# simon-donike/NIR-GAN

Hardware: AMD Instinct MI355X
Metric: 256x256 RGB tiles/sec (G+D fwd+bwd+step) (higher is better)
Workload: dtype f32 (3xbf16 split, 6 products, f32 accumulate) for the contractions with 32-channel runs incl. the Winograd plane GEMMs; exact f32 MFMA for the first / last layers; f32 everywhere else; 1 GPU; configs[1]: 6-block ResnetGenerator + 3-layer PatchGAN, bs=16/GPU, 256x256, GAN+L1, padding=0, fp32-equivalent MFMA (three bf16 terms, six products); global_batch=16, parallelism=dp1

## Files before the change

### nir-gan_amd/csrc/igemm_conv.hip

```cpp
#include "igemm_tiles.h"
#include "igemm_tile256.h"
#include "igemm_x3.h"
#include <cstdlib>
#include "igemm_x3r.h"

namespace {

template <int BN, int PREC = 0, bool WB16 = false, bool AB16 = false>
__global__ __launch_bounds__(256, 2) void conv_igemm_kernel(const ng::ConvParams p) {
    __shared__ __attribute__((aligned(16))) char st0[(128 + BN) * 128];
    __shared__ __attribute__((aligned(16))) char st1[(128 + BN) * 128];
    ng::conv_tile<BN, PREC, WB16, AB16>(p, blockIdx.x, st0, st1);
}

__global__ __launch_bounds__(512, 2) void conv_igemm256_kernel(const ng::ConvParams p) {
    __shared__ __attribute__((aligned(16))) char lds[ng::T256_LDS];
    ng::conv_tile256(p, ng_xcd_remap(blockIdx.x, gridDim.x), lds);
}

template <int BN>
__global__ __launch_bounds__(512, 2) void conv_x3_kernel(const ng::X3Work w) {
    __shared__ __attribute__((aligned(16))) char sA0[ng::X3_A_BYTES];
    __shared__ __attribute__((aligned(16))) char sA1[ng::X3_A_BYTES];
    __shared__ __attribute__((aligned(16))) char sB0[3 * BN * 64];
// ... 51 lines not shown
    int k = 0;
    if (bid >= g.first[1]) k = 1;
    if (bid >= g.first[2]) k = 2;
    if (bid >= g.first[3]) k = 3;
    if (k == 0) ng::conv_tile<BN, PREC, WB16, AB16>(g.p[0], bid, st0, st1);
    else if (k == 1) ng::conv_tile<BN, PREC, WB16, AB16>(g.p[1], bid - g.first[1], st0, st1);
    else if (k == 2) ng::conv_tile<BN, PREC, WB16, AB16>(g.p[2], bid - g.first[2], st0, st1);
    else ng::conv_tile<BN, PREC, WB16, AB16>(g.p[3], bid - g.first[3], st0, st1);
}

}

int ng::ng_cu_count_conv() {
    static int cus = 0;
    if (cus == 0) {
        int dev = 0, n = 0;
        if (hipGetDevice(&dev) != hipSuccess || hipDeviceGetAttribute(&n, hipDeviceAttributeMultiprocessorCount, dev) != hipSuccess || n <= 0) n = 256;
        cus = n;
#ifdef NG_X3R_STAMP
        if (const char* e = getenv("NG_X3R_CUS")) cus = atoi(e);
#endif
    }
    return cus;
}
using ng::ng_cu_count_conv;

int ng::ng_launch_conv_x3(const ng::ConvParams* ps, const int n, const int bn, const int nplanes, const long long in_plane, const long long w3_pstride,
                          const long long out_plane, hipStream_t st, const char* what) {
    ng::X3Work w;
    int total = 0;
    for (int i = 0; i < n; ++i) { w.p[i] = ps[i]; w.first[i] = total; total += ng::conv_x3_tiles(ps[i], bn) * (nplanes > 1 ? nplanes : 1); }
    for (int i = n; i < 4; ++i) { w.p[i] = ps[0]; w.first[i] = 0x7fffffff; }
    w.first[n] = total;
    for (int i = n + 1; i < 5; ++i) w.first[i] = 0x7fffffff;
    w.n = n;
    w.nplanes = nplanes > 1 ? nplanes : 1;
    w.in_plane = in_plane; w.w3_pstride = w3_pstride; w.out_plane = out_plane;
    w.spread = 0;
    for (int i = 0; i < 4; ++i) w.start[i] = 0;
    const int G = ng_cu_count_conv();
    bool unequal = false;
    for (int i = 1; i < n; ++i) unequal = unequal || ps[i].K != ps[0].K;
    if (n >= 2 && w.nplanes == 1 && unequal && total >= G && G <= 1024) {
        long long load[2 * 1024 + 1];
        for (int i = 0; i < G; ++i) load[i] = 0;
        int order[4] = {0, 1, 2, 3};
        for (int i = 0; i < n; ++i)
            for (int j = i + 1; j < n; ++j)
                if (ps[order[j]].K > ps[order[i]].K) { const int t = order[i]; order[i] = order[j]; order[j] = t; }
        for (int oi = 0; oi < n; ++oi) {
            const int k = order[oi];
            const int rem = (w.first[k + 1] - w.first[k]) % G;
            if (rem == 0) continue;
            const long long cost = ps[k].K / 32 + 3;
            long long prefix[2 * 1024 + 1];
            prefix[0] = 0;
            for (int i = 0; i < 2 * G; ++i) prefix[i + 1] = prefix[i] + load[i % G];
            int best = 0;
            for (int s0 = 1; s0 < G; ++s0)
                if (prefix[s0 + rem] - prefix[s0] < prefix[best + rem] - prefix[best]) best = s0;
            for (int t = 0; t < rem; ++t) load[(best + t) % G] += cost;
            w.start[k] = best;
        }
        w.spread = 1;
    }
    const dim3 grid(total < G ? total : G);
    switch (ng::conv_x3_route(ps, n, bn)) {
        case ng::X3R_GENERIC: hipLaunchKernelGGL((conv_x3r_kernel<128, 2>), grid, dim3(256), 0, st, w); break;
        case ng::X3R_STATS: hipLaunchKernelGGL((conv_x3r_kernel<128, 1>), grid, dim3(256), 0, st, w); break;
        case ng::X3R_PLAIN: hipLaunchKernelGGL((conv_x3r_kernel<128, 0>), grid, dim3(256), 0, st, w); break;
        case ng::X3_N128: hipLaunchKernelGGL(conv_x3_kernel<128>, grid, dim3(512), 0, st, w); break;
        case ng::X3_N64: hipLaunchKernelGGL(conv_x3_kernel<64>, grid, dim3(512), 0, st, w); break;
    }
    return nirgan_check_launch(what);
}

ng::X3Kernel ng::conv_x3_route(const ng::ConvParams* ps, const int n, const int bn) {
    bool reg_fed = true, gen = false, stats = false;
    for (int i = 0; i < n; ++i) {
        reg_fed = reg_fed && ng::conv_x3r_ok(ps[i], bn);
        gen = gen || ng::conv_x3r_generic(ps[i]);
        stats = stats || ng::conv_x3r_stats(ps[i]);
    }
    if (reg_fed) return gen ? ng::X3R_GENERIC : (stats ? ng::X3R_STATS : ng::X3R_PLAIN);
    return bn == 128 ? ng::X3_N128 : ng::X3_N64;
}

enum ConvKernel { CONV_K_X3R, CONV_K_X3_N128, CONV_K_X3_N64, CONV_K_TILE256, CONV_K_TILE128, CONV_K_TILE64 };
static const char* const CONV_KERNEL_NAMES[] = {"conv_x3r_kernel<128>", "conv_x3_kernel<128>", "conv_x3_kernel<64>", "conv_igemm256_kernel",
                                                "conv_igemm_kernel<128>", "conv_igemm_kernel<64>"};
struct ConvRoute { ConvKernel k; int bn; };
static ConvRoute conv_route(const ng::ConvParams* ps, const int n, const bool group) {
    bool x3 = ps[0].prec == 3;
    for (int i = 0; i < n; ++i) x3 = x3 && ng::conv_x3_ok(ps[i]) && (ps[i].N % 128 == 0) == (ps[0].N % 128 == 0);
    if (x3) {
        const int bn = ng::conv_x3_bn(ps, n, ng_cu_count_conv());
        const ng::X3Kernel k = ng::conv_x3_route(ps, n, bn);
        return {k == ng::X3_N128 ? CONV_K_X3_N128 : (k == ng::X3_N64 ? CONV_K_X3_N64 : CONV_K_X3R), bn};
    }
    if (!group && ps[0].algo != NIRGAN_CONV_TILE128 && ng::conv_tile256_ok(ps[0])) return {CONV_K_TILE256, 0};
    return {ps[0].N > 64 ? CONV_K_TILE128 : CONV_K_TILE64, 0};
}
static bool conv_route_x3(const ConvRoute& r) { return r.k == CONV_K_X3R || r.k == CONV_K_X3_N128 || r.k == CONV_K_X3_N64; }

#ifdef NG_X3R_STAMP
extern "C" int nirgan_x3r_stamps(unsigned long long* host, int n) {
    return hipMemcpyFromSymbol(host, HIP_SYMBOL(ng::ng_x3r_stamps), size_t(n) * 8) == hipSuccess ? 0 : -1;
}
#endif

extern "C" int nirgan_split3(const float* src, void* dst_bf16, int64_t n, int64_t plane, void* stream) {
    NG_REQUIRE(src && dst_bf16 && n > 0 && n % 8 == 0 && plane >= n && plane % 8 == 0, "split3: n and plane must be positive multiples of 8, plane >= n");
    NG_REQUIRE(ng_aligned16(src) && ng_aligned16(dst_bf16), "split3: pointers must be 16-byte aligned");
    hipLaunchKernelGGL(split3_kernel, dim3((unsigned)((n / 8 + 255) / 256)), dim3(256), 0, static_cast<hipStream_t>(stream),
                       src, static_cast<unsigned short*>(dst_bf16), (long long)n, (long long)plane);
    return nirgan_check_launch("split3");
}

extern "C" int nirgan_conv_igemm(const nirgan_conv_desc* d, void* stream) {
    ng::ConvParams p;
    const int rc = ng::build_conv_params(d, p);
    if (rc != NIRGAN_OK) return rc;
    hipStream_t st = static_cast<hipStream_t>(stream);
    const ConvRoute r = conv_route(&p, 1, false);
    if (conv_route_x3(r)) return ng::ng_launch_conv_x3(&p, 1, r.bn, 1, 0, 0, 0, st, "conv_igemm (three-term split tile)");
    if (p.prec == 3) {
        NG_REQUIRE(p.ch == p.N, "conv: out_span = 2 needs a problem the three-term split tile covers (run %% 32 == 0, N %% 64 == 0)");
        p.prec = 0;
    }
    if (r.k == CONV_K_TILE256) {
        hipLaunchKernelGGL(conv_igemm256_kernel, dim3(((p.M + 255) >> 8) * (p.N >> 8)), dim3(512), 0, st, p);
        return nirgan_check_launch("conv_igemm (256 x 256 tile)");
    }
    const dim3 grid(p.mtiles * p.ntiles * p.ksplit);
    ng::conv_tile_form(p, [&](auto form) {
        using F = decltype(form);
        if (r.k == CONV_K_TILE128) hipLaunchKernelGGL((conv_igemm_kernel<128, F::prec, F::wb16, F::ab16>), grid, dim3(256), 0, st, p);
        else hipLaunchKernelGGL((conv_igemm_kernel<64, F::prec, F::wb16, F::ab16>), grid, dim3(256), 0, st, p);
    });
    if (p.ksplit > 1) {
        const long long total = (long long)p.M * (p.N / 4);
        const int grid = int((total + 255) / 256 < 4096 ? (total + 255) / 256 : 4096);
        hipLaunchKernelGGL(conv_splitk_reduce_kernel, dim3(grid), dim3(256), 0, st, p);
    }
    return nirgan_check_launch("conv_igemm");
}

extern "C" const char* nirgan_conv_kernel_name(const nirgan_conv_desc* d) {
    ng::ConvParams p;
    if (ng::build_conv_params(d, p) != NIRGAN_OK) return nullptr;
    return CONV_KERNEL_NAMES[conv_route(&p, 1, false).k];
}

extern "C" int nirgan_conv_igemm_group(const nirgan_conv_desc* const* descs, int n, void* stream) {
    NG_REQUIRE(descs != nullptr && n >= 1 && n <= 4, "conv_igemm_group: 1..4 descriptors");
    ConvGroup g;
    int total = 0;
    bool wide = false;
    for (int i = 0; i < n; ++i) {
        NG_REQUIRE(descs[i] != nullptr, "conv_igemm_group: null descriptor %d", i);
        const int rc = ng::build_conv_params(descs[i], g.p[i]);
        if (rc != NIRGAN_OK) return rc;
        NG_REQUIRE(descs[i]->ksplit <= 1, "conv_igemm_group: split-K descriptors are not groupable");
        const bool w = descs[i]->N > 64;
        NG_REQUIRE(i == 0 || w == wide, "conv_igemm_group: all problems must use the same tile width (N <= 64 or N > 64)");
        NG_REQUIRE(g.p[i].prec == g.p[0].prec && g.p[i].w_bf16 == g.p[0].w_bf16 && g.p[i].in_bf16 == g.p[0].in_bf16, "conv_igemm_group: all problems must use the same precision and weight storage");
        wide = w;
// ... 23 lines not shown
```

### nir-gan_amd/csrc/igemm_x3r.h

```cpp
#pragma once
#include "igemm_x3.h"

namespace ng {

#ifdef NG_X3R_STAMP
__device__ unsigned long long ng_x3r_stamps[1024 * 4 * 16];
#define X3R_STAMP(k) { unsigned long long t_; __builtin_amdgcn_sched_barrier(0); asm volatile("s_memtime %0\n\ts_waitcnt lgkmcnt(0)" : "=s"(t_) :: "memory"); \
                       __builtin_amdgcn_sched_barrier(0); st_sum[k] += unsigned(t_) - st_last; st_last = unsigned(t_); }
#else
#define X3R_STAMP(k)
#endif

template <int BN>
struct X3R {
    static constexpr int NT = BN / 16;
    static constexpr int B_TERM = BN * 64;
    static constexpr int STAGE = 3 * B_TERM;
    static constexpr int NSTAGE = 2;
    static constexpr int RING = NSTAGE * STAGE;
    static constexpr int STG = 2 * 16 * BN * 4;
    static constexpr int BPT = BN / 16;
    static constexpr int PIECES = 3 * BPT / 4;
    static constexpr int LPR = BN / 4;
    static constexpr int RPP = 64 / LPR;
// ... 360 lines not shown
            asm volatile(X3R_WAITL X3R_PAIR(MA, MA, T, "", "", X3R_ST0, X3R_ST1, "") : X3R_ACC, X3R_B_INOUT, X3R_TERMS : X3R_A_IN, [w] "n"(WAIT), X3R_ST_IN : CLOB); \
        } else if constexpr (WAIT >= 0) { \
            asm volatile(X3R_WAITL X3R_PAIR(MA, MA, T, "", "", "", "", "") : X3R_ACC, X3R_B_INOUT, X3R_TERMS : X3R_A_IN, [w] "n"(WAIT) : CLOB); \
        } else if constexpr (LB) { \
            const char* const lb = P == 0 ? baseW[0] : (P == 1 ? baseW[1] : baseW[2]); \
            const unsigned lo0 = L.b0, lo1 = L.b1; \
            asm volatile(X3R_PAIR(MA, MA, T, "", "", X3R_LB0, X3R_LB1, "") : X3R_ACC, X3R_TERMS, X3R_LB_OUT : X3R_A_IN, X3R_B_IN, [lo0] "v"(lo0), [lo1] "v"(lo1), [lb] "s"(lb) : CLOB); \
        } else if constexpr (LA) { \
            const char* const lb = base; \
            asm volatile(X3R_PAIR(MA, MA, T, "", "", X3R_LA0, X3R_LA1, "") : X3R_ACC, X3R_TERMS, X3R_LA_OUT : X3R_A_IN, X3R_B_IN, [lo0] "v"(goff), [lb] "s"(lb) : CLOB); \
        } else if constexpr (PR) { \
            asm volatile(X3R_PAIR(MA, MA, T, X3R_PR0, X3R_PR1, X3R_PR2, "", "") : X3R_ACC, X3R_TERMS, X3R_PR_OUT : X3R_A_IN, X3R_B_IN, X3R_PR_IN : CLOB); \
        } else { \
            asm volatile(X3R_PAIR(MA, MA, T, "", "", "", "", "") : X3R_ACC, X3R_TERMS : X3R_A_IN, X3R_B_IN : CLOB); \
        }
        if constexpr (P & 1) {
            if constexpr (FIRST) { X3R_EMIT(X3R_MZ, X3R_TB, X3R_CLOB_B) } else { X3R_EMIT(X3R_MC, X3R_TB, X3R_CLOB_B) }
        } else {
            if constexpr (FIRST) { X3R_EMIT(X3R_MZ, X3R_TA, X3R_CLOB_A) } else { X3R_EMIT(X3R_MC, X3R_TA, X3R_CLOB_A) }
        }
#undef X3R_EMIT
#undef X3R_ACC
#undef X3R_B_INOUT
#undef X3R_B_IN
#undef X3R_TERMS
#undef X3R_A_IN
#undef X3R_PR_OUT
#undef X3R_PR_IN
#undef X3R_ST_IN
#undef X3R_LB_OUT
#undef X3R_LA_OUT
        A[SRC][0][P] = h;
        A[SRC][1][P] = m;
        A[SRC][2][P] = l;
    };
#define X3R_RB(NTI, ad) { X3R_DSR(Bf[NTI][0], ad, (NTI) * 1024); X3R_DSR(Bf[NTI][1], ad, B_TERM + (NTI) * 1024); X3R_DSR(Bf[NTI][2], ad, 2 * B_TERM + (NTI) * 1024); }

    struct Slot {
        const NG_CONST ConvParams* p;
        float* out;
        int m0, n0, nk;
    };
    Slot E;
    char* const stg8 = stg_all + wave * T::STG;
    float* const stg = reinterpret_cast<float*>(stg8);
    const unsigned stg_lds = unsigned(size_t((NG_LDS char*)stg8));
    const int chunk = lane % LPR, lrow = lane / LPR;
    struct Epi {
        int pM, OHW, OW, OH, out_img, out_row, out_px, out_org, f_img, f_row, f_px, f_org, pC, span;
        const float* f_y;
        bool fused, stats;
        float fneg;
        int n, nq, nc, m, b, oh, ow, fb, mbase;
        f32x4 bv, fm, fr, s1, s2;
        float k0[NT], t1[NT], t2[NT];
    };
    auto epi_begin = [&](Epi& e) {
#pragma unroll
        for (int nt = 0; nt < NT; ++nt) e.k0[nt] = e.t1[nt] = e.t2[nt] = 0.f;
        const NG_CONST ConvParams& p = *E.p;
        e.pM = p.M; e.OHW = p.OHW; e.OW = p.OW; e.OH = p.OHW / p.OW; e.out_img = p.out_img; e.out_row = p.out_row * p.out_stride;
        e.out_px = p.out_cs * p.out_stride; e.out_org = p.out_org; e.f_img = p.f_img; e.f_row = p.f_row * p.out_stride; e.f_px = p.ch * p.out_stride;
        e.f_org = p.f_org; e.pC = p.ch; e.span = p.N / p.ch;
        e.f_y = p.f_y;
        e.mbase = E.m0 + wave * 64;
        e.fused = e.f_y != nullptr;
        e.stats = p.stats != nullptr && e.mbase < e.pM;
        e.fneg = p.f_act == NIRGAN_ACT_RELU ? 0.f : (p.f_act == NIRGAN_ACT_LRELU ? p.f_slope : 1.f);
        e.n = E.n0 + chunk * 4;
        e.bv = f32x4{0.f, 0.f, 0.f, 0.f};
        if (p.bias != nullptr) {
            const char* bb = ng_uniform_ptr(reinterpret_cast<const char*>(p.bias));
            const unsigned bo = unsigned(e.n) * 4u;
            asm volatile("global_load_dwordx4 %0, %1, %2\n\ts_waitcnt vmcnt(0)" : "=&v"(e.bv) : "v"(bo), "s"(bb) : "memory");
        }
        e.m = e.mbase + lrow;
        const int mc = e.m < e.pM ? e.m : e.pM - 1;
        split_row(mc, e.OHW, e.OW, 1.0f / float(e.OHW), 1.0f / float(e.OW), e.b, e.oh, e.ow);
        e.fb = (e.mbase < e.pM ? e.mbase : e.pM - 1) / e.OHW;
        e.nq = e.n >= e.pC ? 1 : 0;
        e.nc = e.n - e.nq * e.pC;
        e.fm = e.fr = e.s1 = e.s2 = f32x4{0.f, 0.f, 0.f, 0.f};
        if (e.fused) {
            e.fm = *reinterpret_cast<const f32x4*>(p.f_mean + size_t(e.fb) * e.pC + e.nc);
            e.fr = *reinterpret_cast<const f32x4*>(p.f_rstd + size_t(e.fb) * e.pC + e.nc);
        }
    };
    auto stats_acc = [&](Epi& e, auto mt_tag) __attribute__((always_inline)) {
        constexpr int mt = decltype(mt_tag)::value;
#pragma unroll
        for (int nt = 0; nt < NT; ++nt) {
            if constexpr (mt == 0) {
                e.k0[nt] = __shfl(acc[0][nt][0], lane & 15, 64);
                e.t1[nt] = 0.f;
                e.t2[nt] = 0.f;
            }
            const f32x4 c = acc[mt][nt];
            const float c0 = c[0], c1 = c[1], c2 = c[2], c3 = c[3];
            float tmp;
            asm volatile("v_accvgpr_read_b32 %[t], %[c0]\n\tv_sub_f32 %[t], %[t], %[k]\n\tv_add_f32 %[s1], %[s1], %[t]\n\tv_fmac_f32 %[s2], %[t], %[t]\n\t"
                         "v_accvgpr_read_b32 %[t], %[c1]\n\tv_sub_f32 %[t], %[t], %[k]\n\tv_add_f32 %[s1], %[s1], %[t]\n\tv_fmac_f32 %[s2], %[t], %[t]\n\t"
                         "v_accvgpr_read_b32 %[t], %[c2]\n\tv_sub_f32 %[t], %[t], %[k]\n\tv_add_f32 %[s1], %[s1], %[t]\n\tv_fmac_f32 %[s2], %[t], %[t]\n\t"
                         "v_accvgpr_read_b32 %[t], %[c3]\n\tv_sub_f32 %[t], %[t], %[k]\n\tv_add_f32 %[s1], %[s1], %[t]\n\tv_fmac_f32 %[s2], %[t], %[t]"
                         : [t] "=&v"(tmp), [s1] "+v"(e.t1[nt]), [s2] "+v"(e.t2[nt]) : [c0] "a"(c0), [c1] "a"(c1), [c2] "a"(c2), [c3] "a"(c3), [k] "v"(e.k0[nt]));
        }
    };
    auto slice = [&](Epi& e, auto mt_tag, auto mode_tag) __attribute__((always_inline)) {
        constexpr int mt = decltype(mt_tag)::value;
        constexpr bool PLAIN = decltype(mode_tag)::value == 1;
        if (!PLAIN && e.stats) stats_acc(e, mt_tag);
        if constexpr (PLAIN) {
            const unsigned sw = stg_lds + unsigned(((lane >> 4) * 4 * BN + (lane & 15)) * 4);
#pragma unroll
            for (int nt = 0; nt < NT; ++nt)
#pragma unroll
                for (int r = 0; r < 4; ++r) {
                    const float v = acc[mt][nt][r];
                    if (nt == 0) {
                        if (r == 0) asm volatile("ds_write_b32 %0, %1 offset:%2" :: "v"(sw), "a"(v), "n"(0) : "memory");
                        else if (r == 1) asm volatile("ds_write_b32 %0, %1 offset:%2" :: "v"(sw), "a"(v), "n"(BN * 4) : "memory");
                        else if (r == 2) asm volatile("ds_write_b32 %0, %1 offset:%2" :: "v"(sw), "a"(v), "n"(2 * BN * 4) : "memory");
                        else asm volatile("ds_write_b32 %0, %1 offset:%2" :: "v"(sw), "a"(v), "n"(3 * BN * 4) : "memory");
                    }
#define X3R_STW(NTI) else if (nt == NTI) { \
                        if (r == 0) asm volatile("ds_write_b32 %0, %1 offset:%2" :: "v"(sw), "a"(v), "n"(NTI * 64) : "memory"); \
                        else if (r == 1) asm volatile("ds_write_b32 %0, %1 offset:%2" :: "v"(sw), "a"(v), "n"(BN * 4 + NTI * 64) : "memory"); \
                        else if (r == 2) asm volatile("ds_write_b32 %0, %1 offset:%2" :: "v"(sw), "a"(v), "n"(2 * BN * 4 + NTI * 64) : "memory"); \
                        else asm volatile("ds_write_b32 %0, %1 offset:%2" :: "v"(sw), "a"(v), "n"(3 * BN * 4 + NTI * 64) : "memory"); }
                    X3R_STW(1) X3R_STW(2) X3R_STW(3) X3R_STW(4) X3R_STW(5) X3R_STW(6) X3R_STW(7)
#undef X3R_STW
                }
            int ooff[SP];
            bool ok[SP];
#pragma unroll
            for (int pass = 0; pass < SP; ++pass) {
                ok[pass] = e.m < e.pM;
                ooff[pass] = e.b * e.out_img + e.oh * e.out_row + e.ow * e.out_px + e.out_org + e.n;
                e.m += RPP;
                e.ow += RPP;
                const bool wrap_w = e.ow >= e.OW;
                e.ow -= wrap_w ? e.OW : 0;
                e.oh += wrap_w ? 1 : 0;
                const bool wrap_h = e.oh >= e.OH;
                e.oh -= wrap_h ? e.OH : 0;
                e.b += wrap_h ? 1 : 0;
            }
            f32x4 v[SP];
            const unsigned sr = stg_lds + unsigned((lrow * BN + chunk * 4) * 4);
            asm volatile("s_waitcnt lgkmcnt(0)" ::: "memory");
#pragma unroll
            for (int pass = 0; pass < SP; ++pass) asm volatile("ds_read_b128 %0, %1" : "=v"(v[pass]) : "v"(sr + unsigned(pass * RPP * BN * 4)) : "memory");
            if (SP == 8) asm volatile("s_waitcnt lgkmcnt(0)" : "+v"(v[0]), "+v"(v[1]), "+v"(v[2]), "+v"(v[3]), "+v"(v[4 % SP]), "+v"(v[5 % SP]), "+v"(v[6 % SP]), "+v"(v[7 % SP]) :: "memory");
            else asm volatile("s_waitcnt lgkmcnt(0)" : "+v"(v[0]), "+v"(v[1]), "+v"(v[2]), "+v"(v[3]) :: "memory");
#pragma unroll
            for (int pass = 0; pass < SP; ++pass)
                if (ok[pass]) *reinterpret_cast<f32x4*>(E.out + ooff[pass]) = v[pass] + e.bv;
            return;
        }
#pragma unroll
        for (int nt = 0; nt < NT; ++nt)
#pragma unroll
            for (int r = 0; r < 4; ++r) stg[((lane >> 4) * 4 + r) * BN + nt * 16 + (lane & 15)] = acc[mt][nt][r];
        int ooff[SP];
        bool ok[SP];
        f32x4 yv[SP];
#pragma unroll
        for (int pass = 0; pass < SP; ++pass) {
            ok[pass] = e.m < e.pM;
            ooff[pass] = e.b * e.out_img + e.oh * e.out_row + e.ow * e.out_px + e.out_org + e.n;
            if (!PLAIN && e.fused && ok[pass]) yv[pass] = *reinterpret_cast<const f32x4*>(e.f_y + (size_t(e.b) * e.f_img + size_t(e.oh) * e.f_row + size_t(e.ow) * e.f_px + e.f_org + e.n));
            e.m += RPP;
            e.ow += RPP;
            const bool wrap_w = e.ow >= e.OW;
            e.ow -= wrap_w ? e.OW : 0;
            e.oh += wrap_w ? 1 : 0;
            const bool wrap_h = e.oh >= e.OH;
            e.oh -= wrap_h ? e.OH : 0;
            e.b += wrap_h ? 1 : 0;
        }
#pragma unroll
        for (int pass = 0; pass < SP; ++pass) {
            if (ok[pass]) {
                f32x4 v = *reinterpret_cast<const f32x4*>(stg + (pass * RPP + lrow) * BN + chunk * 4);
                v += e.bv;
                *reinterpret_cast<f32x4*>(E.out + ooff[pass]) = v;
                if (!PLAIN && e.fused) {
                    const f32x4 z = (yv[pass] - e.fm) * e.fr;
#pragma unroll
                    for (int q = 0; q < 4; ++q) {
                        const float gz = z[q] > 0.f ? v[q] : v[q] * e.fneg;
                        e.s1[q] += gz;
                        e.s2[q] += gz * z[q];
                    }
                }
            }
        }
    };
    auto stage_w = [&](auto mt_tag, const int only = -1) __attribute__((always_inline)) {
        constexpr int mt = decltype(mt_tag)::value;
        const unsigned sw = stg_lds + unsigned(((lane >> 4) * 4 * BN + (lane & 15)) * 4) + (mt & 1) * (16 * BN * 4), sw2 = sw + 2 * BN * 4;
#pragma unroll
        for (int nt = 0; nt < NT; ++nt) {
            if ((only >= 0 && nt != only) || (NG_X3R_KO & 32)) continue;
            const f32x4 c = acc[mt][nt];
            const float c0 = c[0], c1 = c[1], c2 = c[2], c3 = c[3];
#define X3R_STW4(NTI) if (nt == NTI) asm volatile("ds_write2_b32 %0, %2, %3 offset0:%6 offset1:%7\n\tds_write2_b32 %1, %4, %5 offset0:%6 offset1:%7" \
                    :: "v"(sw), "v"(sw2), "a"(c0), "a"(c1), "a"(c2), "a"(c3), "n"(NTI * 16), "n"(NTI * 16 + BN) : "memory");
            X3R_STW4(0) X3R_STW4(1) X3R_STW4(2) X3R_STW4(3) X3R_STW4(4) X3R_STW4(5) X3R_STW4(6) X3R_STW4(7)
#undef X3R_STW4
        }
    };
    auto epilogue_full = [&](Epi& e, auto bias_tag, auto&& mid) __attribute__((always_inline)) {
        constexpr bool BIAS = decltype(bias_tag)::value;
        const unsigned sr0 = stg_lds + unsigned((lrow * BN + chunk * 4) * 4);
        constexpr unsigned HALF = 16 * BN * 4;
        const char* const obase = ng_uniform_ptr(reinterpret_cast<const char*>(E.out));
        const unsigned d0 = unsigned(RPP * e.out_px) * 4u, dW = unsigned(e.out_row - e.OW * e.out_px) * 4u, dH = unsigned(e.out_img - e.OH * e.out_row) * 4u;
        unsigned off = unsigned(e.b * e.out_img + e.oh * e.out_row + e.ow * e.out_px + e.out_org + e.n) * 4u;
        int s_ow = __builtin_amdgcn_readfirstlane(e.ow);
        const int s_OW = e.OW;
        static_assert(7 * 16 + BN <= 255, "ds_write2_b32 offsets are 8-bit dword counts");
        f32x4 v0[SP], v1[SP];
        auto R = [&](auto mt_tag, f32x4 (&vv)[SP]) __attribute__((always_inline)) {
            constexpr int mt = decltype(mt_tag)::value;
            const unsigned sr = sr0 + (mt & 1) * HALF;
#pragma unroll
            for (int pass = 0; pass < SP; ++pass) {
                if (NG_X3R_KO & 32) { asm volatile("" : "=v"(vv[pass]) :: "memory"); continue; }
                if (pass == 0) asm volatile("ds_read_b128 %0, %1" : "=v"(vv[0]) : "v"(sr) : "memory");
#define X3R_RDP(P) else if (pass == P) asm volatile("ds_read_b128 %0, %1 offset:%2" : "=v"(vv[P % SP]) : "v"(sr), "n"(P * RPP * BN * 4) : "memory");
                X3R_RDP(1) X3R_RDP(2) X3R_RDP(3) X3R_RDP(4) X3R_RDP(5) X3R_RDP(6) X3R_RDP(7)
#undef X3R_RDP
            }
        };
        auto Aoff = [&](unsigned (&ooff)[SP]) __attribute__((always_inline)) {
            if (s_ow + 16 <= s_OW) {
#pragma unroll
                for (int pass = 0; pass < SP; ++pass) ooff[pass] = off + pass * d0;
                off += SP * d0;
                e.ow += 16;
                const bool wrap_w = e.ow >= e.OW;
                e.ow -= wrap_w ? e.OW : 0;
                off += wrap_w ? dW : 0;
                e.oh += wrap_w ? 1 : 0;
                const bool wrap_h = e.oh >= e.OH;
                e.oh -= wrap_h ? e.OH : 0;
                off += wrap_h ? dH : 0;
                s_ow += 16;
                s_ow -= s_ow >= s_OW ? s_OW : 0;
            } else {
#pragma unroll
                for (int pass = 0; pass < SP; ++pass) {
                    ooff[pass] = off;
                    off += d0;
                    e.ow += RPP;
                    const bool wrap_w = e.ow >= e.OW;
                    e.ow -= wrap_w ? e.OW : 0;
                    off += wrap_w ? dW : 0;
                    e.oh += wrap_w ? 1 : 0;
                    const bool wrap_h = e.oh >= e.OH;
                    e.oh -= wrap_h ? e.OH : 0;
                    off += wrap_h ? dH : 0;
                }
                s_ow += 16;
                s_ow -= s_ow >= s_OW ? s_OW : 0;
            }
        };
        auto S = [&](auto next_tag, f32x4 (&vv)[SP], const unsigned (&ooff)[SP]) __attribute__((always_inline)) {
            constexpr int NEXT = decltype(next_tag)::value;
            if constexpr (false) {
                if (SP == 8) asm volatile("s_waitcnt lgkmcnt(15)" : "+v"(vv[0]), "+v"(vv[1]), "+v"(vv[2]), "+v"(vv[3]), "+v"(vv[4 % SP]), "+v"(vv[5 % SP]), "+v"(vv[6 % SP]), "+v"(vv[7 % SP]) :: "memory");
                else asm volatile("s_waitcnt lgkmcnt(15)" : "+v"(vv[0]), "+v"(vv[1]), "+v"(vv[2]), "+v"(vv[3]) :: "memory");
            } else {
                if (SP == 8) asm volatile("s_waitcnt lgkmcnt(0)" : "+v"(vv[0]), "+v"(vv[1]), "+v"(vv[2]), "+v"(vv[3]), "+v"(vv[4 % SP]), "+v"(vv[5 % SP]), "+v"(vv[6 % SP]), "+v"(vv[7 % SP]) :: "memory");
                else asm volatile("s_waitcnt lgkmcnt(0)" : "+v"(vv[0]), "+v"(vv[1]), "+v"(vv[2]), "+v"(vv[3]) :: "memory");
            }
            const char* const ob = obase;
            if constexpr (BIAS) {
#pragma unroll
                for (int pass = 0; pass < SP; ++pass) vv[pass] += e.bv;
            }
            static_assert(SP == NT, "one column block of the next slice per store");
#pragma unroll
            for (int pass = 0; pass < SP; ++pass) {
                const unsigned oo = ooff[pass];
                if (!(NG_X3R_KO & 64)) asm volatile("global_store_dwordx4 %1, %0, %2" : "+v"(vv[pass]) : "v"(oo), "s"(ob) : "memory");
                if constexpr (NEXT < 4) stage_w(next_tag, pass);
            }
            asm volatile("s_nop 1" :: "v"(vv[0]), "v"(vv[1]), "v"(vv[2]), "v"(vv[3]), "v"(vv[4 % SP]), "v"(vv[5 % SP]), "v"(vv[6 % SP]), "v"(vv[7 % SP]) : "memory");
        };
        using J0 = std::integral_constant<int, 0>; using J1 = std::integral_constant<int, 1>; using J2 = std::integral_constant<int, 2>; using J3 = std::integral_constant<int, 3>;
        using J4 = std::integral_constant<int, 4>;
        unsigned oo[SP];
        Aoff(oo); R(J0{}, v0); S(J1{}, v0, oo);
        Aoff(oo); R(J1{}, v1); S(J2{}, v1, oo);
        mid();
        Aoff(oo); R(J2{}, v0); S(J3{}, v0, oo);
        Aoff(oo); R(J3{}, v1); S(J4{}, v1, oo);
    };
    auto stats_flush = [&](Epi& e) __attribute__((always_inline)) {
        const NG_CONST ConvParams& p = *E.p;
        const int b = e.mbase / e.OHW;
        float* sp = p.stats + (size_t(b) * p.stats_cps + p.stats_chunk0 + ((e.mbase - b * e.OHW) >> 6) * e.span) * 4 * e.pC;
        const char* const sb8 = ng_uniform_ptr(reinterpret_cast<const char*>(sp));
        const int field = lane >> 4;
#pragma unroll
        for (int nt = 0; nt < NT; ++nt) {
            float s1 = e.t1[nt], s2 = e.t2[nt];
            s1 += __shfl_xor(s1, 16, 64);
            s2 += __shfl_xor(s2, 16, 64);
            s1 += __shfl_xor(s1, 32, 64);
            s2 += __shfl_xor(s2, 32, 64);
            int col = E.n0 + nt * 16 + (lane & 15);
            if (col >= e.pC) col += 3 * e.pC;
            const float val = field == 0 ? e.k0[nt] : (field == 1 ? s1 : (field == 2 ? s2 : 64.f));
            const unsigned so = unsigned(field * e.pC + col) * 4u;
            asm volatile("global_store_dword %0, %1, %2" :: "v"(so), "v"(val), "s"(sb8) : "memory");
        }
    };
    auto epi_finish = [&](Epi& e) {
        const NG_CONST ConvParams& p = *E.p;
        if (e.stats) {
            const int b = e.mbase / e.OHW;
            float* sp = p.stats + (size_t(b) * p.stats_cps + p.stats_chunk0 + ((e.mbase - b * e.OHW) >> 6) * e.span) * 4 * e.pC;
#pragma unroll
            for (int nt = 0; nt < NT; ++nt) {
                float s1 = e.t1[nt], s2 = e.t2[nt];
                s1 += __shfl_xor(s1, 16, 64);
                s2 += __shfl_xor(s2, 16, 64);
                s1 += __shfl_xor(s1, 32, 64);
                s2 += __shfl_xor(s2, 32, 64);
                int col = E.n0 + nt * 16 + (lane & 15);
                if (col >= e.pC) col += 3 * e.pC;
                if (lane < 16) {
                    sp[col] = e.k0[nt];
                    sp[e.pC + col] = s1;
                    sp[2 * e.pC + col] = s2;
                    sp[3 * e.pC + col] = 64.f;
                }
            }
        }
        if (e.fused) {
#pragma unroll
            for (int q = 0; q < 4; ++q)
#pragma unroll
                for (int o = LPR; o < 64; o <<= 1) {
                    e.s1[q] += __shfl_xor(e.s1[q], o, 64);
                    e.s2[q] += __shfl_xor(e.s2[q], o, 64);
                }
            f32x4* const red = reinterpret_cast<f32x4*>(sRed);
            if (lane < LPR) {
                red[(wave * LPR + chunk) * 2] = e.s1;
                red[(wave * LPR + chunk) * 2 + 1] = e.s2;
            }
            asm volatile("s_waitcnt lgkmcnt(0)" ::: "memory");
            __builtin_amdgcn_s_barrier();
            asm volatile("" ::: "memory");
            if ((wave & 1) == 0 && lane < LPR && e.mbase < e.pM) {
                const f32x4 t1 = e.s1 + red[((wave + 1) * LPR + chunk) * 2], t2 = e.s2 + red[((wave + 1) * LPR + chunk) * 2 + 1];
                float* pp = p.f_part + (size_t(e.fb) * p.f_cps + p.f_chunk0 + ((e.mbase - e.fb * e.OHW) >> 7) * e.span + e.nq) * 2 * e.pC + e.nc;
                *reinterpret_cast<f32x4*>(pp) = t1;
                *reinterpret_cast<f32x4*>(pp + e.pC) = t2;
            }
            asm volatile("s_waitcnt lgkmcnt(0)" ::: "memory");
            __builtin_amdgcn_s_barrier();
            asm volatile("" ::: "memory");
        }
    };

    auto tile = [&](auto first_tag) __attribute__((always_inline)) {
        const unsigned bnext = ring0 + unsigned((sj ^ 1) * STAGE) + b_rd;
        const unsigned stage_next = unsigned((sj ^ 1) * STAGE);
        auto block = [&](auto mt_tag, auto src_tag, const char* base, const unsigned goff) __attribute__((always_inline)) {
            constexpr int MT = decltype(mt_tag)::value, SRC = decltype(src_tag)::value;
            if (MT == 0) {
                if constexpr (decltype(first_tag)::value) {
                    const int sb = __builtin_amdgcn_readfirstlane(stores_behind);
                    if (PIECES == 6) asm volatile(X3R_WAITV2(6) : "+v"(Braw[0]), "+v"(Braw[1]), "+v"(Braw[2]), "+v"(Braw[3 % PIECES]), "+v"(Braw[4 % PIECES]), "+v"(Braw[5 % PIECES]) : [sb] "s"(sb), [n1] "n"(6 + EST), [n2] "n"(6 + EST + NT) : "memory", "scc");
                    else asm volatile(X3R_WAITV2(6) : "+v"(Braw[0]), "+v"(Braw[1]), "+v"(Braw[2]) : [sb] "s"(sb), [n1] "n"(6 + EST), [n2] "n"(6 + EST + NT) : "memory", "scc");
                } else {
                    if (PIECES == 6) asm volatile("s_waitcnt vmcnt(6)" : "+v"(Braw[0]), "+v"(Braw[1]), "+v"(Braw[2]), "+v"(Braw[3 % PIECES]), "+v"(Braw[4 % PIECES]), "+v"(Braw[5 % PIECES]) :: "memory");
                    else asm volatile("s_waitcnt vmcnt(6)" : "+v"(Braw[0]), "+v"(Braw[1]), "+v"(Braw[2]) :: "memory");
                }
            }
            wait_raw(F[SRC], std::integral_constant<int, MT == 1 ? 6 : 12>{}, first_tag);
            auto one = [&](auto p_tag) __attribute__((always_inline)) {
                constexpr int P = decltype(p_tag)::value, nt = 2 * P + 1;
                static_assert(NT == 8, "the 64-column form needs its own region");
                constexpr int behind = 3 * (NT - 1 - nt);
                using W = std::integral_constant<int, MT == 0 ? (behind > 15 ? 15 : behind) : -1>;
                region(first_tag, mt_tag, p_tag, src_tag, W{}, bnext, b_wr + stage_next, base, goff);
                if constexpr (MT == 2 && P < 3) step_early(std::integral_constant<int, P + 1>{});
                if constexpr (MT == 3 && P == 3) {
                    X3R_RB(6, bnext)
                    X3R_RB(7, bnext)
                    if (!(NG_X3R_KO & 4)) loadA(F[SRC], base, goff);
                }
                if (MT == 3 && P == 3) { sj ^= 1; step_cursor(); }
            };
            static_assert(PIECES == 6, "six B pieces per wave and K-tile: two behind each of three regions");
            one(std::integral_constant<int, 0>{}); one(std::integral_constant<int, 1>{}); one(std::integral_constant<int, 2>{}); one(std::integral_constant<int, 3>{});
        };
        using I0 = std::integral_constant<int, 0>; using I1 = std::integral_constant<int, 1>; using I2 = std::integral_constant<int, 2>; using I3 = std::integral_constant<int, 3>;
        X3R_STAMP(5)
        block(I0{}, I3{}, baseP, goff3P);
        X3R_STAMP(0)
        block(I1{}, I0{}, baseC, L.goff[0]);
        X3R_STAMP(1)
        step_early(std::integral_constant<int, 0>{});
        asm volatile("s_waitcnt lgkmcnt(0)" ::: "memory");
        __builtin_amdgcn_s_barrier();
        asm volatile("" ::: "memory");
        __builtin_amdgcn_sched_barrier(0);
        X3R_STAMP(2)
        block(I2{}, I1{}, baseC, L.goff[1]);
        X3R_STAMP(3)
        block(I3{}, I2{}, baseC, L.goff[2]);
        X3R_STAMP(4)
#ifdef NG_X3R_STAMP
        ++st_sum[15];
#endif
    };

    auto keep = [&](const Item& t, Slot& q) { q.p = t.p; q.out = t.out; q.m0 = t.m0; q.n0 = t.n0; q.nk = t.nk; };
    {
        Item t;
        locate(itemN, t);
        if (t.nk < 0) return;
        prepare(t, N);
        keep(t, E);
    }
    L = N;
    left = L.nk;
    Slot Q1, Q2;
    auto prepare_next = [&]() {
        Item t;
        locate(itemN + G, t);
        Q2.nk = t.nk;
        if (t.nk >= 0) {
            itemN += G;
            prepare(t, N);
            keep(t, Q2);
        }
    };
    prepare_next();
    Q1 = Q2;
    cursor_bases();
    loadA(F[0], baseC, L.goff[0]);
    loadA(F[1], baseC, L.goff[1]);
    loadA(F[2], baseC, L.goff[2]);
#pragma unroll
    for (int i = 0; i < PIECES; ++i) loadB(i);
    if (PIECES == 6) asm volatile("s_waitcnt vmcnt(0)" : "+v"(Braw[0]), "+v"(Braw[1]), "+v"(Braw[2]), "+v"(Braw[3 % PIECES]), "+v"(Braw[4 % PIECES]), "+v"(Braw[5 % PIECES]),
                                  "+v"(F[0][0]), "+v"(F[0][1]), "+v"(F[1][0]), "+v"(F[1][1]), "+v"(F[2][0]), "+v"(F[2][1]) :: "memory");
    else asm volatile("s_waitcnt vmcnt(0)" : "+v"(Braw[0]), "+v"(Braw[1]), "+v"(Braw[2]), "+v"(F[0][0]), "+v"(F[0][1]), "+v"(F[1][0]), "+v"(F[1][1]), "+v"(F[2][0]), "+v"(F[2][1]) :: "memory");
#pragma unroll
    for (int i = 0; i < PIECES; ++i) storeB(0u, i);
#pragma unroll
    for (int i = 0; i < 4; ++i) { convert_pair(F[0], A[0], i); convert_pair(F[1], A[1], i); convert_pair(F[2], A[2], i); }
    asm volatile("s_waitcnt lgkmcnt(0)" ::: "memory");
    __builtin_amdgcn_s_barrier();
    asm volatile("" ::: "memory");
    {
        const unsigned b0 = ring0 + b_rd;
#pragma unroll
        for (int nt = 0; nt < NT; ++nt) {
            if (nt == 0) X3R_RB(0, b0) else if (nt == 1) X3R_RB(1, b0) else if (nt == 2) X3R_RB(2, b0) else if (nt == 3) X3R_RB(3, b0)
            else if (nt == 4) X3R_RB(4 % NT, b0) else if (nt == 5) X3R_RB(5 % NT, b0) else if (nt == 6) X3R_RB(6 % NT, b0) else X3R_RB(7 % NT, b0)
        }
    }
    loadA(F[3], baseC, L.goff[3]);
    step_cursor();
#pragma unroll
    for (int i = 0; i < PIECES; ++i) loadB(i);
    loadA(F[0], baseC, L.goff[0]);
    loadA(F[1], baseC, L.goff[1]);
    loadA(F[2], baseC, L.goff[2]);
    step_cursor();
#ifdef NG_X3R_STAMP
    { unsigned long long t_; asm volatile("s_memtime %0\n\ts_waitcnt lgkmcnt(0)" : "=s"(t_) :: "memory"); st_last = unsigned(t_); }
#endif
    int nkC = E.nk;
    using I0 = std::integral_constant<int, 0>; using I1 = std::integral_constant<int, 1>; using I2 = std::integral_constant<int, 2>; using I3 = std::integral_constant<int, 3>;
    while (true) {
        tile(std::true_type{});
        stores_behind = 0;
        for (int k = 1; k < nkC; ++k) tile(std::false_type{});
        X3R_STAMP(9)
        X3R_MFMA_DRAIN;
        if constexpr (GEN) {
            static_assert(PIECES == 6, "six raw B pieces per wave");
            asm volatile("s_waitcnt vmcnt(0)" : "+v"(F[0][0]), "+v"(F[0][1]), "+v"(F[1][0]), "+v"(F[1][1]), "+v"(F[2][0]), "+v"(F[2][1]), "+v"(F[3][0]), "+v"(F[3][1]),
                         "+v"(Braw[0]), "+v"(Braw[1]), "+v"(Braw[2]), "+v"(Braw[3 % PIECES]), "+v"(Braw[4 % PIECES]), "+v"(Braw[5 % PIECES]) :: "memory");
        }
        Epi e;
        bool full = false;
        if constexpr (KIND == 0) {
            full = E.m0 + 256 <= E.p->M;
            if (full) stage_w(I0{});
        }
        epi_begin(e);
        X3R_STAMP(6)
        if constexpr (!GEN) {
            bool st = false;
            if constexpr (STATS) {
                full = E.m0 + 256 <= e.pM;
                st = e.stats;
                if (st) { stats_acc(e, I0{}); stats_acc(e, I1{}); stats_acc(e, I2{}); stats_acc(e, I3{}); stats_flush(e); }
                if (full) stage_w(I0{});
            }
            if (full) {
                if (E.p->bias != nullptr) epilogue_full(e, std::true_type{}, prepare_next); else epilogue_full(e, std::false_type{}, prepare_next);
                stores_behind = st ? 2 : 1;
            } else {
                slice(e, I0{}, I1{});
                slice(e, I1{}, I1{});
                slice(e, I2{}, I1{});
                slice(e, I3{}, I1{});
                prepare_next();
            }
        } else {
            slice(e, I0{}, I2{});
            slice(e, I1{}, I2{});
            slice(e, I2{}, I2{});
            slice(e, I3{}, I2{});
            epi_finish(e);
            prepare_next();
        }
        X3R_STAMP(7)
#ifdef NG_X3R_STAMP
        ++st_sum[14];
#endif
        E = Q1;
        Q1 = Q2;
        if (E.nk < 0) break;
        nkC = E.nk;
        X3R_STAMP(8)
    }
#ifdef NG_X3R_STAMP
    {
        unsigned long long c1, r1;
        asm volatile("s_memtime %0\n\ts_memrealtime %1\n\ts_waitcnt lgkmcnt(0)" : "=s"(c1), "=s"(r1) :: "memory");
        st_sum[12] = unsigned(c1 - st_c0);
        st_sum[13] = unsigned(r1 - st_r0);
    }
    if (lane == 0 && blockIdx.x < 1024) {
#pragma unroll
        for (int i = 0; i < 16; ++i) ng_x3r_stamps[(blockIdx.x * 4 + wave) * 16 + i] = st_sum[i];
    }
#endif
#undef X3R_RB
}
#undef X3R_GLD
#undef X3R_WAITV2
#undef X3R_VALU
#undef X3R_DSR

inline bool conv_x3r_generic(const ConvParams& p) { return p.f_y != nullptr; }
inline bool conv_x3r_stats(const ConvParams& p) { return p.stats != nullptr; }
#ifndef NG_X3R_GEN_MIN_NK
#define NG_X3R_GEN_MIN_NK 24
#endif
inline bool conv_x3r_ok(const ConvParams& p, const int bn) {
    const int nk = p.ntaps * (p.run >> 5);
    return bn == 128 && p.algo == NIRGAN_CONV_X3_R4 && p.OW >= 16 && nk >= (conv_x3r_generic(p) ? NG_X3R_GEN_MIN_NK : 3)
           && p.out_elems * 4 <= (1ll << 32) && p.M < (1 << 24);
}

}
```

Measured before the change: 1086 tiles/s.

## Add full-tile fused norm-backward epilogue to register-fed x3 conv generic path

Gives the generic (fused normalization-backward) path of the register-fed x3r conv kernel a full-tile epilogue. It streams f_y loads alongside the output stores and accumulates the gradient statistics in inline asm; partial tiles fall back to a rolled per-row loop. It lowers the generic-path minimum K from 24 to 3 while routing short, small-grid generic convs and mixed gen+stats batches to the old x3 kernel, and drops the in-kernel stats write from the generic finish. This aims to move more fused backward convs onto the faster register-fed kernel, at the cost of more register pressure, more routing heuristics and a 32-bit offset limit on f_y.

```diff
diff --git a/nir-gan_amd/csrc/igemm_conv.hip b/nir-gan_amd/csrc/igemm_conv.hip
--- a/nir-gan_amd/csrc/igemm_conv.hip
+++ b/nir-gan_amd/csrc/igemm_conv.hip
@@ -157,7 +157,14 @@
         gen = gen || ng::conv_x3r_generic(ps[i]);
         stats = stats || ng::conv_x3r_stats(ps[i]);
     }
-    if (reg_fed) return gen ? ng::X3R_GENERIC : (stats ? ng::X3R_STATS : ng::X3R_PLAIN);
+    long long tiles = 0;
+    bool short_gen = false;
+    for (int i = 0; i < n; ++i) {
+        tiles += ng::conv_x3_tiles(ps[i], bn);
+        short_gen = short_gen || (ng::conv_x3r_generic(ps[i]) && ps[i].ntaps * (ps[i].run >> 5) < NG_X3R_GEN_FULL_NK);
+    }
+    if (short_gen && tiles < ng_cu_count_conv()) reg_fed = false;
+    if (reg_fed && !(gen && stats)) return gen ? ng::X3R_GENERIC : (stats ? ng::X3R_STATS : ng::X3R_PLAIN);
     return bn == 128 ? ng::X3_N128 : ng::X3_N64;
 }
 
diff --git a/nir-gan_amd/csrc/igemm_x3r.h b/nir-gan_amd/csrc/igemm_x3r.h
--- a/nir-gan_amd/csrc/igemm_x3r.h
+++ b/nir-gan_amd/csrc/igemm_x3r.h
@@ -466,8 +466,10 @@
         e.nc = e.n - e.nq * e.pC;
         e.fm = e.fr = e.s1 = e.s2 = f32x4{0.f, 0.f, 0.f, 0.f};
         if (e.fused) {
-            e.fm = *reinterpret_cast<const f32x4*>(p.f_mean + size_t(e.fb) * e.pC + e.nc);
-            e.fr = *reinterpret_cast<const f32x4*>(p.f_rstd + size_t(e.fb) * e.pC + e.nc);
+            const char* mb = ng_uniform_ptr(reinterpret_cast<const char*>(p.f_mean));
+            const char* rb = ng_uniform_ptr(reinterpret_cast<const char*>(p.f_rstd));
+            const unsigned fo = unsigned(e.fb * e.pC + e.nc) * 4u;
+            asm volatile("global_load_dwordx4 %0, %2, %3\n\tglobal_load_dwordx4 %1, %2, %4\n\ts_waitcnt vmcnt(0)" : "=&v"(e.fm), "=&v"(e.fr) : "v"(fo), "s"(mb), "s"(rb) : "memory");
         }
     };
     auto stats_acc = [&](Epi& e, auto mt_tag) __attribute__((always_inline)) {
@@ -594,13 +596,16 @@
 #undef X3R_STW4
         }
     };
-    auto epilogue_full = [&](Epi& e, auto bias_tag, auto&& mid) __attribute__((always_inline)) {
-        constexpr bool BIAS = decltype(bias_tag)::value;
+    auto epilogue_full = [&](Epi& e, auto bias_tag, auto fused_tag, auto&& mid) __attribute__((always_inline)) {
+        constexpr bool BIAS = decltype(bias_tag)::value, FUSED = decltype(fused_tag)::value;
         const unsigned sr0 = stg_lds + unsigned((lrow * BN + chunk * 4) * 4);
         constexpr unsigned HALF = 16 * BN * 4;
         const char* const obase = ng_uniform_ptr(reinterpret_cast<const char*>(E.out));
         const unsigned d0 = unsigned(RPP * e.out_px) * 4u, dW = unsigned(e.out_row - e.OW * e.out_px) * 4u, dH = unsigned(e.out_img - e.OH * e.out_row) * 4u;
         unsigned off = unsigned(e.b * e.out_img + e.oh * e.out_row + e.ow * e.out_px + e.out_org + e.n) * 4u;
+        const unsigned y0 = unsigned(RPP * e.f_px) * 4u, yW = unsigned(e.f_row - e.OW * e.f_px) * 4u, yH = unsigned(e.f_img - e.OH * e.f_row) * 4u;
+        unsigned yoff = unsigned(e.b * e.f_img + e.oh * e.f_row + e.ow * e.f_px + e.f_org + e.n) * 4u;
+        const char* const ybase = ng_uniform_ptr(reinterpret_cast<const char*>(e.f_y));
         int s_ow = __builtin_amdgcn_readfirstlane(e.ow);
         const int s_OW = e.OW;
         static_assert(7 * 16 + BN <= 255, "ds_write2_b32 offsets are 8-bit dword counts");
@@ -617,19 +622,26 @@
 #undef X3R_RDP
             }
         };
-        auto Aoff = [&](unsigned (&ooff)[SP]) __attribute__((always_inline)) {
+        auto Aoff = [&](unsigned (&ooff)[SP], unsigned (&yo)[SP]) __attribute__((always_inline)) {
             if (s_ow + 16 <= s_OW) {
 #pragma unroll
                 for (int pass = 0; pass < SP; ++pass) ooff[pass] = off + pass * d0;
                 off += SP * d0;
+                if constexpr (FUSED) {
+#pragma unroll
+                    for (int pass = 0; pass < SP; ++pass) yo[pass] = yoff + pass * y0;
+                    yoff += SP * y0;
+                }
                 e.ow += 16;
                 const bool wrap_w = e.ow >= e.OW;
                 e.ow -= wrap_w ? e.OW : 0;
                 off += wrap_w ? dW : 0;
+                if constexpr (FUSED) yoff += wrap_w ? yW : 0;
                 e.oh += wrap_w ? 1 : 0;
                 const bool wrap_h = e.oh >= e.OH;
                 e.oh -= wrap_h ? e.OH : 0;
                 off += wrap_h ? dH : 0;
+                if constexpr (FUSED) yoff += wrap_h ? yH : 0;
                 s_ow += 16;
                 s_ow -= s_ow >= s_OW ? s_OW : 0;
             } else {
@@ -637,14 +649,17 @@
                 for (int pass = 0; pass < SP; ++pass) {
                     ooff[pass] = off;
                     off += d0;
+                    if constexpr (FUSED) { yo[pass] = yoff; yoff += y0; }
                     e.ow += RPP;
                     const bool wrap_w = e.ow >= e.OW;
                     e.ow -= wrap_w ? e.OW : 0;
                     off += wrap_w ? dW : 0;
+                    if constexpr (FUSED) yoff += wrap_w ? yW : 0;
                     e.oh += wrap_w ? 1 : 0;
                     const bool wrap_h = e.oh >= e.OH;
                     e.oh -= wrap_h ? e.OH : 0;
                     off += wrap_h ? dH : 0;
+                    if constexpr (FUSED) yoff += wrap_h ? yH : 0;
                 }
                 s_ow += 16;
                 s_ow -= s_ow >= s_OW ? s_OW : 0;
@@ -673,14 +688,83 @@
             }
             asm volatile("s_nop 1" :: "v"(vv[0]), "v"(vv[1]), "v"(vv[2]), "v"(vv[3]), "v"(vv[4 % SP]), "v"(vv[5 % SP]), "v"(vv[6 % SP]), "v"(vv[7 % SP]) : "memory");
         };
+        f32x4 yv[SP];
+        auto Y = [&](const unsigned (&yo)[SP]) __attribute__((always_inline)) {
+            if constexpr (FUSED) {
+                const char* const yb = ybase;
+#pragma unroll
+                for (int pass = 0; pass < SP; ++pass) {
+                    const unsigned o = yo[pass];
+                    asm volatile("global_load_dwordx4 %0, %1, %2" : "=&v"(yv[pass]) : "v"(o), "s"(yb) : "memory");
+                }
+            }
+        };
+        auto Z = [&](const f32x4 (&vv)[SP]) __attribute__((always_inline)) {
+            if constexpr (FUSED) {
+                static_assert(SP == 8, "eight row segments per slice");
+                asm volatile("s_waitcnt vmcnt(8)" : "+v"(yv[0]), "+v"(yv[1]), "+v"(yv[2]), "+v"(yv[3]), "+v"(yv[4 % SP]), "+v"(yv[5 % SP]), "+v"(yv[6 % SP]), "+v"(yv[7 % SP]) :: "memory");
+                const float m0 = e.fm[0], m1 = e.fm[1], m2 = e.fm[2], m3 = e.fm[3], r0 = e.fr[0], r1 = e.fr[1], r2 = e.fr[2], r3 = e.fr[3], fn = e.fneg;
+                float a0 = e.s1[0], a1 = e.s1[1], a2 = e.s1[2], a3 = e.s1[3], b0 = e.s2[0], b1 = e.s2[1], b2 = e.s2[2], b3 = e.s2[3];
+#pragma unroll
+                for (int pass = 0; pass < SP; ++pass) {
+                    const float y_0 = yv[pass][0], y_1 = yv[pass][1], y_2 = yv[pass][2], y_3 = yv[pass][3];
+                    const float v_0 = vv[pass][0], v_1 = vv[pass][1], v_2 = vv[pass][2], v_3 = vv[pass][3];
+                    float z, w, t;
+#define X3R_FZ0(Q, Z) "v_sub_f32 %[" #Z "], %[y" #Q "], %[m" #Q "]\n\t"
+#define X3R_FZ1(Q, Z, GAP) "v_mul_f32 %[" #Z "], %[" #Z "], %[r" #Q "]\n\tv_cmp_lt_f32 vcc, 0, %[" #Z "]\n\tv_mul_f32 %[t], %[v" #Q "], %[fn]\n\t" GAP \
+                           "v_cndmask_b32 %[t], %[t], %[v" #Q "], vcc\n\tv_add_f32 %[a" #Q "], %[a" #Q "], %[t]\n\tv_fmac_f32 %[b" #Q "], %[t], %[" #Z "]\n\t"
+                    asm volatile(X3R_FZ0(0, z) X3R_FZ1(0, z, X3R_FZ0(1, w)) X3R_FZ1(1, w, X3R_FZ0(2, z)) X3R_FZ1(2, z, X3R_FZ0(3, w)) X3R_FZ1(3, w, "s_nop 0\n\t")
+                                 : [z] "=&v"(z), [w] "=&v"(w), [t] "=&v"(t), [a0] "+v"(a0), [a1] "+v"(a1), [a2] "+v"(a2), [a3] "+v"(a3), [b0] "+v"(b0), [b1] "+v"(b1), [b2] "+v"(b2), [b3] "+v"(b3)
+                                 : [y0] "v"(y_0), [y1] "v"(y_1), [y2] "v"(y_2), [y3] "v"(y_3), [v0] "v"(v_0), [v1] "v"(v_1), [v2] "v"(v_2), [v3] "v"(v_3),
+                                   [m0] "v"(m0), [m1] "v"(m1), [m2] "v"(m2), [m3] "v"(m3), [r0] "v"(r0), [r1] "v"(r1), [r2] "v"(r2), [r3] "v"(r3), [fn] "v"(fn)
+                                 : "vcc");
+#undef X3R_FZ0
+#undef X3R_FZ1
+                }
+                e.s1 = f32x4{a0, a1, a2, a3};
+                e.s2 = f32x4{b0, b1, b2, b3};
+            }
+        };
         using J0 = std::integral_constant<int, 0>; using J1 = std::integral_constant<int, 1>; using J2 = std::integral_constant<int, 2>; using J3 = std::integral_constant<int, 3>;
         using J4 = std::integral_constant<int, 4>;
-        unsigned oo[SP];
-        Aoff(oo); R(J0{}, v0); S(J1{}, v0, oo);
-        Aoff(oo); R(J1{}, v1); S(J2{}, v1, oo);
+        unsigned oo[SP], yo[SP];
+        Aoff(oo, yo); Y(yo); R(J0{}, v0); S(J1{}, v0, oo); Z(v0);
+        Aoff(oo, yo); Y(yo); R(J1{}, v1); S(J2{}, v1, oo); Z(v1);
         mid();
-        Aoff(oo); R(J2{}, v0); S(J3{}, v0, oo);
-        Aoff(oo); R(J3{}, v1); S(J4{}, v1, oo);
+        Aoff(oo, yo); Y(yo); R(J2{}, v0); S(J3{}, v0, oo); Z(v0);
+        Aoff(oo, yo); Y(yo); R(J3{}, v1); S(J4{}, v1, oo); Z(v1);
+    };
+    auto slice_rolled = [&](Epi& e, auto mt_tag) __attribute__((always_inline)) {
+        constexpr int mt = decltype(mt_tag)::value;
+        stage_w(mt_tag);
+        asm volatile("s_waitcnt lgkmcnt(0)" ::: "memory");
+        const float* const half = stg + (mt & 1) * (16 * BN) + lrow * BN + chunk * 4;
+#pragma unroll 1
+        for (int pass = 0; pass < SP; ++pass) {
+            if (e.m < e.pM) {
+                f32x4 v = *reinterpret_cast<const f32x4*>(half + pass * RPP * BN);
+                v += e.bv;
+                *reinterpret_cast<f32x4*>(E.out + (e.b * e.out_img + e.oh * e.out_row + e.ow * e.out_px + e.out_org + e.n)) = v;
+                if (e.fused) {
+                    const f32x4 yy = *reinterpret_cast<const f32x4*>(e.f_y + (size_t(e.b) * e.f_img + size_t(e.oh) * e.f_row + size_t(e.ow) * e.f_px + e.f_org + e.n));
+                    const f32x4 z = (yy - e.fm) * e.fr;
+#pragma unroll
+                    for (int q = 0; q < 4; ++q) {
+                        const float gz = z[q] > 0.f ? v[q] : v[q] * e.fneg;
+                        e.s1[q] += gz;
+                        e.s2[q] += gz * z[q];
+                    }
+                }
+            }
+            e.m += RPP;
+            e.ow += RPP;
+            const bool wrap_w = e.ow >= e.OW;
+            e.ow -= wrap_w ? e.OW : 0;
+            e.oh += wrap_w ? 1 : 0;
+            const bool wrap_h = e.oh >= e.OH;
+            e.oh -= wrap_h ? e.OH : 0;
+            e.b += wrap_h ? 1 : 0;
+        }
     };
     auto stats_flush = [&](Epi& e) __attribute__((always_inline)) {
         const NG_CONST ConvParams& p = *E.p;
@@ -704,26 +788,6 @@
     };
     auto epi_finish = [&](Epi& e) {
         const NG_CONST ConvParams& p = *E.p;
-        if (e.stats) {
-            const int b = e.mbase / e.OHW;
-            float* sp = p.stats + (size_t(b) * p.stats_cps + p.stats_chunk0 + ((e.mbase - b * e.OHW) >> 6) * e.span) * 4 * e.pC;
-#pragma unroll
-            for (int nt = 0; nt < NT; ++nt) {
-                float s1 = e.t1[nt], s2 = e.t2[nt];
-                s1 += __shfl_xor(s1, 16, 64);
-                s2 += __shfl_xor(s2, 16, 64);
-                s1 += __shfl_xor(s1, 32, 64);
-                s2 += __shfl_xor(s2, 32, 64);
-                int col = E.n0 + nt * 16 + (lane & 15);
-                if (col >= e.pC) col += 3 * e.pC;
-                if (lane < 16) {
-                    sp[col] = e.k0[nt];
-                    sp[e.pC + col] = s1;
-                    sp[2 * e.pC + col] = s2;
-                    sp[3 * e.pC + col] = 64.f;
-                }
-            }
-        }
         if (e.fused) {
 #pragma unroll
             for (int q = 0; q < 4; ++q)
@@ -872,15 +936,14 @@
         for (int k = 1; k < nkC; ++k) tile(std::false_type{});
         X3R_STAMP(9)
         X3R_MFMA_DRAIN;
-        if constexpr (GEN) {
-            static_assert(PIECES == 6, "six raw B pieces per wave");
-            asm volatile("s_waitcnt vmcnt(0)" : "+v"(F[0][0]), "+v"(F[0][1]), "+v"(F[1][0]), "+v"(F[1][1]), "+v"(F[2][0]), "+v"(F[2][1]), "+v"(F[3][0]), "+v"(F[3][1]),
-                         "+v"(Braw[0]), "+v"(Braw[1]), "+v"(Braw[2]), "+v"(Braw[3 % PIECES]), "+v"(Braw[4 % PIECES]), "+v"(Braw[5 % PIECES]) :: "memory");
-        }
         Epi e;
         bool full = false;
         if constexpr (KIND == 0) {
             full = E.m0 + 256 <= E.p->M;
+            if (full) stage_w(I0{});
+        }
+        if constexpr (GEN) {
+            full = E.m0 + 256 <= E.p->M && E.p->f_y != nullptr && E.p->bias == nullptr;
             if (full) stage_w(I0{});
         }
         epi_begin(e);
@@ -894,7 +957,7 @@
                 if (full) stage_w(I0{});
             }
             if (full) {
-                if (E.p->bias != nullptr) epilogue_full(e, std::true_type{}, prepare_next); else epilogue_full(e, std::false_type{}, prepare_next);
+                if (E.p->bias != nullptr) epilogue_full(e, std::true_type{}, std::false_type{}, prepare_next); else epilogue_full(e, std::false_type{}, std::false_type{}, prepare_next);
                 stores_behind = st ? 2 : 1;
             } else {
                 slice(e, I0{}, I1{});
@@ -904,12 +967,21 @@
                 prepare_next();
             }
         } else {
-            slice(e, I0{}, I2{});
-            slice(e, I1{}, I2{});
-            slice(e, I2{}, I2{});
-            slice(e, I3{}, I2{});
-            epi_finish(e);
-            prepare_next();
+            if (full) {
+                epilogue_full(e, std::false_type{}, std::true_type{}, prepare_next);
+                stores_behind = 1;
+                epi_finish(e);
+            } else {
+                static_assert(PIECES == 6, "six raw B pieces per wave");
+                asm volatile("s_waitcnt vmcnt(0)" : "+v"(F[0][0]), "+v"(F[0][1]), "+v"(F[1][0]), "+v"(F[1][1]), "+v"(F[2][0]), "+v"(F[2][1]), "+v"(F[3][0]), "+v"(F[3][1]),
+                             "+v"(Braw[0]), "+v"(Braw[1]), "+v"(Braw[2]), "+v"(Braw[3 % PIECES]), "+v"(Braw[4 % PIECES]), "+v"(Braw[5 % PIECES]) :: "memory");
+                slice_rolled(e, I0{});
+                slice_rolled(e, I1{});
+                slice_rolled(e, I2{});
+                slice_rolled(e, I3{});
+                epi_finish(e);
+                prepare_next();
+            }
         }
         X3R_STAMP(7)
 #ifdef NG_X3R_STAMP
@@ -943,12 +1015,16 @@
 inline bool conv_x3r_generic(const ConvParams& p) { return p.f_y != nullptr; }
 inline bool conv_x3r_stats(const ConvParams& p) { return p.stats != nullptr; }
 #ifndef NG_X3R_GEN_MIN_NK
-#define NG_X3R_GEN_MIN_NK 24
+#define NG_X3R_GEN_MIN_NK 3
+#endif
+#ifndef NG_X3R_GEN_FULL_NK
+#define NG_X3R_GEN_FULL_NK 24
 #endif
 inline bool conv_x3r_ok(const ConvParams& p, const int bn) {
     const int nk = p.ntaps * (p.run >> 5);
+    const bool y_ok = !conv_x3r_generic(p) || (long long)(p.M / p.OHW) * p.f_img * 4 <= (1ll << 32);
     return bn == 128 && p.algo == NIRGAN_CONV_X3_R4 && p.OW >= 16 && nk >= (conv_x3r_generic(p) ? NG_X3R_GEN_MIN_NK : 3)
-           && p.out_elems * 4 <= (1ll << 32) && p.M < (1 << 24);
+           && p.out_elems * 4 <= (1ll << 32) && p.M < (1 << 24) && y_ok;
 }
 
 }
```

New measurement: 1093 tiles/s, median of 6. No clear change (+0.6%).
